# Inuri04/pgtg

Hardware: NVIDIA B200
Metric: env-steps/sec (higher is better)
Workload: dtype int32+f64

## Files before the change

### pgtg_b200/csrc/pgtg_api_impl.hpp

```cpp
#pragma once
#include <math.h>
#include <stdio.h>
#include <stdlib.h>
#include <string.h>

#include <string>
#include <vector>

#include "pgtg_phases.cuh"

using namespace pgtg;

#include "pgtg_env.hpp"

#ifdef PGTG_BACKEND_LEVELS
static const bool bk_has_levels = true;
#else
static const bool bk_has_levels = false;
static int bk_serve_levels(pgtg_env*, void*) { return -1; }
static int bk_levels(pgtg_env*, int32_t*, int, void*) { return -1; }
#endif
#ifdef PGTG_BACKEND_OBS_BITS
static const bool bk_has_obs_bits = true;
#else
// ... 170 lines not shown
  d.visited_penalty = c.already_visited_position_penalty;
  d.ice_p = c.ice_probability; d.broken_p = c.street_damage_probability; d.sand_p = c.sand_probability;
  d.traffic_density = c.traffic_density;
  d.light_green = c.light_green; d.light_yellow = c.light_yellow; d.light_total = c.light_green + c.light_yellow + c.light_red;
  d.ignore_traffic_collisions = c.ignore_traffic_collisions;
  for (int i = 0; i < 5; i++) {
    d.profile_cdf[i] = c.profile_cdf[i]; d.drv_yellow_stop[i] = c.drv_yellow_stop[i]; d.drv_red_violation[i] = c.drv_red_violation[i];
    d.drv_patience_threshold[i] = c.drv_patience_threshold[i]; d.drv_push_probability[i] = c.drv_push_probability[i];
    d.drv_speed_multiplier[i] = c.drv_speed_multiplier[i]; d.drv_reaction_delay[i] = c.drv_reaction_delay[i];
    d.drv_min_following[i] = c.drv_min_following[i];
  }
  d.separate_reward_cost = c.separate_reward_cost; d.num_rules = c.num_rules; d.max_episode_steps = c.max_episode_steps;
  d.write_final_obs = c.write_final_obs;
  for (int i = 0; i < c.num_rules; i++) if (c.rules[i].min_traffic <= 0 && c.rules[i].min_matching_traffic <= 0) d.rules_without_traffic = 1;
  d.max_cars = c.max_cars > 0 ? c.max_cars : 1;
  d.lut_radius = (d.WS > d.HS ? d.WS : d.HS) + 2;
  int words = (d.T + 1) / 2;
  if ((words & 1) == 0) words++;
  d.tile_stride = words * 2;
  for (int t = 0; t < d.T; t++) {
    if (t % d.W < d.W - 1) d.full_e[t >> 5] |= 1u << (t & 31);
    if (t + d.W < d.T) d.full_s[t >> 5] |= 1u << (t & 31);
  }
  if (c.already_visited_position_penalty != 0) { d.vis_w = d.HS + 2; d.vis_words = ((d.WS + 2) * (d.HS + 2) + 31) / 32; }
  d.obs_bits = d.C * d.P * d.P;
  if (c.traffic_density > 0) { d.occ_words = (d.WS * d.HS + 15) / 16;   d.spawner_cap = 2 * (d.W + d.H) + d.T; }
  d.pregen = (c.rng_mode != PGTG_RNG_TAPE && !c.fixed_map) ? 1 : 0;
  d.lean = lean_predicate(c, d);
  d.env_id_base = c.env_id_base; d.seed = c.seed;
  d.num_levels = c.num_levels; d.level_sampling = c.level_sampling; d.start_level = c.start_level;
  if (!c.fixed_map) {
    d.n_edge_tab = 2 * (d.W * (d.H - 1) + d.H * (d.W - 1));
    d.n_border_slots = 2 * d.W + 2 * d.H - 2;
    int n_he = d.H * (d.W - 1), n_ve = d.W * (d.H - 1);
    if (c.start_mode == 0 && c.goal_mode == 0 && d.T <= 32 && n_he + n_ve >= 1 && n_he + n_ve <= bk_conn_table_max_bits() &&
        !(c.start_x == c.goal_x && c.start_y == c.goal_y)) {
      d.conn_bits = n_he + n_ve; d.conn_ne = n_he;
      d.path_tab = d.T <= 16 ? 1 : 0;
    }
    int n_slots = 2 * d.W + 2 * d.H - 2;
    if (c.border_connections < 0 || c.border_connections > n_slots) { why = "random_map_percentage_of_connections must be in [0, 1]"; return -1; }
    if (c.edges_to_keep < 0) { why = "random_map_percentage_of_connections must be in [0, 1]"; return -1; }
  }
  return 0;
}

static int build_level_pool(pgtg_env* e) {
  const size_t M = (size_t)e->cfg.num_levels, T = (size_t)e->dc.T;
  DevPtrs& p = e->dp;
  if (!(p.level_tiles = dev_alloc<uint16_t>(e, M * T + 8, false)) || !(p.level_plan = dev_alloc<uint32_t>(e, M, false))) return -1;
  uint16_t* ring = (uint16_t*)bk_alloc(2 * M * T * 2 + 16);
  uint32_t* plans = (uint32_t*)bk_alloc(2 * M * 4);
  uint64_t* keys = (uint64_t*)bk_alloc(M * 8);
  uint2* list = (uint2*)bk_alloc(2 * M * sizeof(uint2));
  uint32_t* count = (uint32_t*)bk_alloc(8);
  uint32_t* err = (uint32_t*)bk_alloc(M * 4);
  int rc = (ring && plans && keys && list && count && err) ? 0 : -1;
  if (!rc) {
    std::vector<uint64_t> hk(M);
    std::vector<uint2> hl(M);
    for (size_t j = 0; j < M; j++) { hk[j] = (uint64_t)e->cfg.start_level + j; hl[j].x = (uint32_t)j; hl[j].y = 1u; }
    const uint32_t hc[2] = {(uint32_t)M, 0u};
    rc = bk_h2d(keys, hk.data(), M * 8, nullptr) || bk_h2d(list, hl.data(), M * sizeof(uint2), nullptr) || bk_h2d(count, hc, 8, nullptr) ||
         bk_memset(err, 0, M * 4) || bk_sync(nullptr);
  }
  if (!rc) {
// ... 12 lines not shown
    std::vector<uint32_t> hp(M);
    rc = bk_d2d(p.level_tiles, ring + M * T, M * T * 2, nullptr) || bk_d2h(hp.data(), plans + M, M * 4, nullptr) || bk_sync(nullptr);
    for (size_t j = 0; j < M; j++) hp[j] &= ~(3u << 29);
    rc = rc || bk_h2d(p.level_plan, hp.data(), M * 4, nullptr) || bk_sync(nullptr);
  }
  for (void* a : {(void*)ring, (void*)plans, (void*)keys, (void*)list, (void*)count, (void*)err}) if (a) bk_free(a);
  return rc;
}

static int32_t level_fingerprint(const pgtg_config& c) {
  if (!c.num_levels) return 0;
  uint32_t h = 0x9E3779B9u;
  h = (h ^ (uint32_t)c.num_levels) * 0x85EBCA6Bu;
  h = (h ^ (uint32_t)c.start_level) * 0xC2B2AE35u;
  h = (h ^ (uint32_t)c.level_sampling) * 0x27D4EB2Fu;
  return (int32_t)(h | 1u);
}

extern "C" int pgtg_create(const pgtg_config* cfg, int device, pgtg_env** out) {
  if (!cfg || !out) return fail(PGTG_ERR_INVALID, "null argument");
  *out = nullptr;
  DevCfg dc;
  std::string why;
  if (fill_devcfg(*cfg, dc, why)) return fail(PGTG_ERR_INVALID, why);
  if (cfg->num_levels && !bk_has_levels) return fail(PGTG_ERR_INVALID, "num_levels: this backend has no level sets");
  if (bk_set_device(device)) return fail(PGTG_ERR_CUDA, std::string("cannot select device: ") + bk_error());
  pgtg_env* e = new pgtg_env();
  e->cfg = *cfg; e->dc = dc; e->device = device; e->launches = 0;
  e->max_steps_cfg = dc.max_episode_steps; e->gamma_cap = 0;
  e->have_fixed = e->have_tape = e->did_reset = false;
  e->cars_injected = false;
  e->timing = false; e->tev_used = 0;
  e->side_stream = e->ev_tick = e->ev_map[0] = e->ev_map[1] = nullptr;
  e->launch_index = 0; e->mapgen_grid = 0; e->inline_mapgen = false;
  e->flat = nullptr; e->flat_dim = 0;
  e->info_dev = nullptr;
  e->packed_dev = nullptr; e->stage_dev[0] = e->stage_dev[1] = nullptr; e->stage_bytes = 0; e->copy_stream = nullptr;
  e->ev_stage[0] = e->ev_stage[1] = e->ev_copied[0] = e->ev_copied[1] = nullptr; e->host_steps = 0;
  e->obs_format = PGTG_OBS_INT8; e->obs_map_buf = e->f_obs_map_buf = nullptr; e->obs_packed_buf = e->f_obs_packed_buf = nullptr;
  memset(&e->dp, 0, sizeof e->dp);
  if (pick_block(e->dc, &e->block, &e->smem)) { delete e; return fail(PGTG_ERR_INVALID, "observation window too large for shared memory"); }
  e->nblk = (dc.N + e->block - 1) / e->block;
  e->stats_rows = nullptr;
  e->traffic_G = e->traffic_NT = 0;
  const bool wants_traffic_tick = cfg->traffic_density > 0 || ((cfg->sliding || cfg->use_next_subgoal_direction) && !cfg->fixed_map && getenv("PGTG_TRAFFIC_KERNEL_CARFREE"));
  if (cfg->rng_mode == PGTG_RNG_PHILOX && wants_traffic_tick && !getenv("PGTG_NO_TRAFFIC_KERNEL")) bk_traffic_geometry(e->dc, &e->traffic_G, &e->traffic_NT);
  e->stats_nrows = e->nblk;
  if (e->traffic_G > 0 && (dc.N + e->traffic_G - 1) / e->traffic_G > e->stats_nrows) e->stats_nrows = (dc.N + e->traffic_G - 1) / e->traffic_G;
  DevPtrs& p = e->dp;
  size_t N = (size_t)dc.N;
  bool ok = true;
#define A(field, type, count) ok = ok && ((p.field = dev_alloc<type>(e, (count))) != nullptr) && (e->state_allocs.push_back({p.field, sizeof(type) * (size_t)(count)}), true)
  A(agent, short4, N); A(misc, uint32_t, N); A(elapsed, uint32_t, N); A(episode, uint32_t, N); A(next_car_id, uint32_t, N);
  A(plan, uint32_t, N); A(tiles, uint16_t, N * dc.T + 8);
  if (dc.pregen) { A(next_tiles, uint16_t, 2 * N * dc.T + 8); A(next_plan, uint32_t, 2 * N); A(regen_list, uint2, 4 * N); A(regen_count, uint32_t, 4); } A(cars, uint64_t, 2 * (size_t)dc.max_cars * N);
  if (dc.vis_words) A(visited, uint32_t, (size_t)dc.vis_words * N);
  if (dc.occ_words) { A(occ, uint32_t, (size_t)dc.occ_words * N); A(spawners, uint16_t, (size_t)dc.spawner_cap * N); A(spawner_count, uint16_t, N); }
  A(key, uint64_t, N); A(error, uint32_t, N); A(ep_return, double, N);
  if (cfg->rng_mode == PGTG_RNG_TAPE) { A(cursor, int64_t, N); A(tape_end, int64_t, N); }
  if (cfg->rng_mode == PGTG_RNG_NUMPY) { A(pcg, PcgState, 4 * N); p.pcg_stride = N; }
  A(obs_map, int8_t, N * dc.obs_bits + 16); A(obs_position, int32_t, 2 * N); A(obs_velocity, int32_t, 2 * N); A(obs_nsd, int32_t, N);
  A(reward, double, N); A(cost, double, N); A(terminated, uint8_t, N); A(truncated, uint8_t, N);
  A(step_state, int32_t, 4 * N); A(step_flags, uint8_t, N);
  if (dc.write_final_obs) {
    A(f_obs_map, int8_t, N * dc.obs_bits + 16); A(f_obs_position, int32_t, 2 * N); A(f_obs_velocity, int32_t, 2 * N); A(f_obs_nsd, int32_t, N);
  }
  A(stats, double, 8);
// ... 66 lines not shown
          uint8_t& v = tl[((size_t)ex * 81 + sq) * PGTG_NUM_ROUTE_IDS + r];
          if ((l & 7) != 0) v |= (uint8_t)(16u << ((l & 7) - 1));
          for (int i = 0; i < (int)((l >> 3) & 7); i++)
            if ((int)((l >> (6 + 7 * i)) & 31) == r) v |= (uint8_t)(1u << ((l >> (11 + 7 * i)) & 3));
        }
      }
    uint8_t* sd = dev_alloc<uint8_t>(e, sl.size());
    uint8_t* tdv = dev_alloc<uint8_t>(e, tl.size());
    if (!sd || !tdv) { pgtg_destroy(e); return fail(PGTG_ERR_CUDA, "device allocation failed"); }
    bk_h2d(sd, sl.data(), sl.size(), nullptr);
    bk_h2d(tdv, tl.data(), tl.size(), nullptr);
    bk_sync(nullptr);
    p.step_lut = sd; p.target_lut = tdv;
  }
  {
    std::vector<uint8_t> lut;
    build_direction_lut(dc.lut_radius, lut);
    uint8_t* d = dev_alloc<uint8_t>(e, lut.size());
    pgtg_rule* r = dev_alloc<pgtg_rule>(e, PGTG_MAX_RULES);
    if (!d || !r) { pgtg_destroy(e); return fail(PGTG_ERR_CUDA, "device allocation failed"); }
    bk_h2d(d, lut.data(), lut.size(), nullptr);
    bk_h2d(r, cfg->rules, sizeof(pgtg_rule) * PGTG_MAX_RULES, nullptr);
    p.dirlut = d; p.rules = r;
  }
  if (e->dc.pregen) {
    int sms = 0;
    if (bk_side_create(&e->side_stream, &e->ev_tick, &e->ev_map[0], &e->ev_map[1], &sms)) {
      pgtg_destroy(e);
      return fail(PGTG_ERR_CUDA, std::string("cannot create the map-generation stream: ") + bk_error());
    }
    const char* env_ctas = getenv("PGTG_MAPGEN_CTAS_PER_SM");
    int per_sm = env_ctas ? atoi(env_ctas) : 0;
    e->mapgen_grid = per_sm > 0 ? sms * per_sm : 0;
    e->mapgen_grid_overlap = e->mapgen_grid; e->overlap = !getenv("PGTG_NO_OVERLAP");
    e->inline_mapgen = bk_inline_mapgen() && getenv("PGTG_INLINE_MAPGEN") != nullptr && cfg->rng_mode == PGTG_RNG_PHILOX && !getenv("PGTG_NO_LEAN") && !cfg->num_levels;
  }
  if (e->dc.conn_bits) {
    size_t words = ((size_t)1 << e->dc.conn_bits) / 32 + 1;
    uint32_t* t = dev_alloc<uint32_t>(e, words, false);
    if (!t || bk_build_conn_table(e, t)) { pgtg_destroy(e); return fail(PGTG_ERR_CUDA, std::string("connectivity table: ") + bk_error()); }
    p.conn_table = t;
    const int W = e->dc.W, H = e->dc.H, n_he = H * (W - 1);
    std::vector<uint2> ft((size_t)e->dc.conn_bits);
    for (auto& m : ft) m.x = m.y = 0x80000000u;
    auto add = [&](int edge, uint32_t others) { uint2& m = ft[(size_t)edge]; if (m.x == 0x80000000u) m.x = others; else m.y = others; };
    for (int r = 0; r + 1 < H; r++)
      for (int x = 0; x + 1 < W; x++) {
        const int f[4] = {r * (W - 1) + x, (r + 1) * (W - 1) + x, n_he + r * W + x, n_he + r * W + x + 1};
        uint32_t all = 0;
        for (int k = 0; k < 4; k++) all |= 1u << f[k];
        for (int k = 0; k < 4; k++) add(f[k], all & ~(1u << f[k]));
      }
    uint2* fd = dev_alloc<uint2>(e, ft.size());
    if (!fd) { pgtg_destroy(e); return fail(PGTG_ERR_CUDA, "device allocation failed"); }
    bk_h2d(fd, ft.data(), ft.size() * sizeof(uint2), nullptr);
    p.face_tab = fd;
  }
  if (e->dc.path_tab) {
    uint64_t* t = dev_alloc<uint64_t>(e, (size_t)1 << e->dc.conn_bits, false);
    if (!t || bk_build_path_table(e, t)) { pgtg_destroy(e); return fail(PGTG_ERR_CUDA, std::string("path table: ") + bk_error()); }
    p.path_table = t;
  }
  if (!pgtg::map_in_registers(e->dc)) e->inline_mapgen = false;
  if (cfg->num_levels && build_level_pool(e)) { pgtg_destroy(e); return fail(PGTG_ERR_CUDA, std::string("level pool: ") + bk_error()); }
  bk_sync(nullptr);
  *out = e;
// ... 733 lines not shown
```

### pgtg_b200/csrc/pgtg_device.cuh

```cuda
#pragma once
#include <stdint.h>
#include <stdlib.h>

#ifdef __CUDACC__
#include <cuda_runtime.h>
#define PG_HD __device__ __forceinline__
#define PG_HDN static __device__ __noinline__
#define PG_HOSTDEV __host__ __device__ inline
#define PG_MEMBER __device__
#define PG_DEVCONST __device__ const
#define pg_umulhi(a, b) __umulhi((a), (b))
#define pg_ffs(v) __ffs((int)(v))
#define pg_popc(v) __popc((unsigned)(v))
#define pg_clz(v) __clz((int)(v))
#define pg_popcll(v) __popcll((unsigned long long)(v))
#define pg_ldg(p) __ldg(p)
#define pg_dmul(a, b) __dmul_rn((a), (b))
#define pg_dadd(a, b) __dadd_rn((a), (b))
#define pg_ddiv(a, b) __ddiv_rn((a), (b))
#define pg_atomic_or(p, v) atomicOr((p), (v))
#define pg_atomic_add(p, v) atomicAdd((p), (v))
#define pg_atomic_cas(p, o, n) atomicCAS((p), (o), (n))
#define pg_atomic_min(p, v) atomicMin((p), (v))
#define pg_store_streaming(ptr, v) __stcs((ptr), (v))
// ... 101 lines not shown
}
PG_HOSTDEV unsigned car_xy(uint64_t v) { return (unsigned)(v & 0xFFFF); }

struct DevCfg {
  int N, W, H, T, WS, HS;
  int C, P, sliding, window_k, use_nsd;
  int channel_kind[PGTG_MAX_CHANNELS];
  int kind_channel[16];
  int lean;
  int obs_fast;
  int fixed_map, edges_to_keep, n_edge_tab, border_connections, n_border_slots;
  int start_mode, goal_mode, start_x, start_y, start_dir, goal_x, goal_y, goal_dir, min_sg_dist;
  double obstacle_probability, obstacle_cdf[4];
  double sum_subgoals_reward, final_goal_bonus, crash_penalty, light_penalty, standing_penalty, visited_penalty;
  double ice_p, broken_p, sand_p, traffic_density;
  int light_green, light_yellow, light_total, ignore_traffic_collisions;
  double profile_cdf[5], drv_yellow_stop[5], drv_red_violation[5], drv_patience_threshold[5], drv_push_probability[5],
      drv_speed_multiplier[5], drv_reaction_delay[5];
  int drv_min_following[5];
  int separate_reward_cost, num_rules, max_episode_steps, write_final_obs, max_cars, lut_radius;
  int pregen;
  int rules_without_traffic;
  int tile_stride;
  int vis_w, vis_words;
  int occ_words, spawner_cap;
  int obs_bits;
  uint32_t full_e[8], full_s[8];
  int conn_bits, conn_ne;
  int path_tab;
  int eval_on, gamma_len;
  int64_t env_id_base;
  uint64_t seed;
  int num_levels, level_sampling, start_level;
};

struct PcgState {
  uint64_t st_lo, st_hi, inc_lo, inc_hi;
  uint32_t buf, has;
};

struct Lut;

struct DevPtrs {
  short4* agent;
  uint32_t* misc;
  uint32_t* elapsed;
  uint32_t* episode;
  uint32_t* next_car_id;
  uint32_t* plan;
  uint16_t* tiles;
  uint16_t* next_tiles;
  uint32_t* next_plan;
  uint2* regen_list;
  uint32_t* regen_count;
  int parity;
  uint64_t* cars;
  uint32_t* visited;
  uint32_t* occ;
  uint16_t* spawners;
  uint16_t* spawner_count;
  uint64_t* key;
  PcgState* pcg;
  size_t pcg_stride;
  int64_t* cursor;
  int64_t* tape_end;
  const double* tape_values;
// ... 406 lines not shown
```

### pgtg_b200/csrc/pgtg_env.hpp

```cpp
#pragma once
#include <stdint.h>

#include <vector>

#include "pgtg_phases.cuh"

using namespace pgtg;

namespace pgtg { constexpr int STATS_STRIDE = 8; }

enum { MODE_STEP = 0, MODE_RESET = 1, MODE_OBSERVE = 2, MODE_MAPGEN = 3 };

struct pgtg_env {
  pgtg_config cfg;
  DevCfg dc;
  DevPtrs dp;
  int device;
  int block;
  size_t smem;
  int64_t launches;
  std::vector<void*> allocs;
  struct StateAlloc { void* ptr; size_t bytes; };
  std::vector<StateAlloc> state_allocs;
  bool have_fixed, have_tape, did_reset;
  int max_steps_cfg;
  int gamma_cap;
  bool cars_injected;
  int nblk;
  int stats_nrows;
  int traffic_G, traffic_NT;
  void* side_stream; void* ev_tick; void* ev_map[2];
  uint64_t launch_index;
  bool inline_mapgen;
  int mapgen_grid;
  int mapgen_grid_overlap; bool overlap;
  bool timing; std::vector<void*> tev; int tev_used;
  float* flat; int flat_dim; int flat_order[PGTG_MAX_CHANNELS];
  uint32_t* packed_dev; unsigned char* stage_dev[2]; size_t stage_bytes; void* copy_stream; void* ev_stage[2]; void* ev_copied[2]; uint64_t host_steps;
  int obs_format; int8_t* obs_map_buf; int8_t* f_obs_map_buf; uint32_t* obs_packed_buf; uint32_t* f_obs_packed_buf;
  uint32_t* unpack_err;
  int32_t* info_dev;
  double* stats_rows;
  uint8_t* mask_dev;
  int64_t* seeds_dev;
  int32_t* actions_dev;
  std::vector<uint16_t> edge_tab, edge_rev, border_slots;
};

static inline bool inline_mapgen_now(const pgtg_env* e) { return e->inline_mapgen && e->dc.pregen && e->dc.lean == 1 && !e->dc.write_final_obs; }
```

### pgtg_b200/csrc/pgtg_logic.cuh

```cuda
#pragma once
#include "pgtg_device.cuh"

namespace pgtg {

PG_HD int select32(uint32_t v, int n);

PG_HD uint64_t* car_list(const DevCfg& c, const DevPtrs& p, int env, int half) { return p.cars + ((size_t)env * 2 + half) * c.max_cars; }

PG_HD int light_phase(const DevCfg& c, int counter) {
  return counter < c.light_green ? 0 : (counter < c.light_green + c.light_yellow ? 1 : 2);
}

PG_HD void or_bit81(uint32_t w[3], int sq) {
  uint32_t b = 1u << (sq & 31);
  int i = sq >> 5;
  w[0] |= i == 0 ? b : 0u; w[1] |= i == 1 ? b : 0u; w[2] |= i == 2 ? b : 0u;
}

PG_HD void spawner_bits(const DevCfg& c, const Lut& L, int ex, int tx, int ty, uint32_t out[3]) {
  out[0] = out[1] = out[2] = 0;
  if (ex == 0) return;
  int ns = L.native_spawner[ex];
  if (ns != 255) or_bit81(out, ns);
  if (tx == 0) { int sq = L.entry_sq[3]; if (ld_all(lane_desc(ex, sq)) == 4) or_bit81(out, sq); }
// ... 585 lines not shown

template <int RNG>
PG_HD uint32_t remove_edges_tabled(const DevCfg& c, const DevPtrs& p, Rng<RNG>& rng, uint8_t* arr) {
  const int n_und = c.H * (c.W - 1) + c.W * (c.H - 1);
  uint32_t graph = (c.conn_bits >= 32 ? 0u : (1u << c.conn_bits)) - 1u;
  for (int i = 0; 4 * i < n_und; i++) ((uint32_t*)arr)[i] = 0x03020100u + 0x04040404u * (uint32_t)i;
  int n = n_und;
  int go = n > 0 ? 2 * n_und - c.edges_to_keep : 0;
  uint32_t pos = rng.position(PGTG_STREAM_MAP);
  while (go > 0) {
    uint32_t w[4];
    rng.block(PGTG_STREAM_MAP, pos >> 2, w);
#pragma unroll
    for (int k = 0; k < 4; k++) {
      if (go > 0) {
        const int i = (int)pg_umulhi(w[k], (uint32_t)n);
        const int edge = arr[i];
        const uint32_t pbit = 1u << edge;
        arr[i] = arr[n - 1];
        n--; pos++;
        const uint32_t g2 = graph & ~pbit;
        const uint2 face = pg_ldg(&p.face_tab[edge]);
        bool keep = (graph & face.x) == face.x || (graph & face.y) == face.y;
        if (!keep) keep = (pg_ldg(&p.conn_table[g2 >> 5]) >> (g2 & 31)) & 1u;
        graph = keep ? g2 : graph;
        go = n > 0 ? 2 * pg_popc(graph) - c.edges_to_keep : 0;
      }
    }
  }
  rng.set_position(PGTG_STREAM_MAP, pos);
  return graph;
}

template <int RNG, typename MASK = uint64_t>
PG_HD MASK choose_border_slots(const DevCfg& c, Rng<RNG>& rng) {
  const int n = c.n_border_slots;
  int left = c.border_connections < n ? c.border_connections : n;
  MASK chosen = 0;
  if (left <= 0) return chosen;
  const int cbits = edge_chunk_bits(n), per_word = 32 / cbits;
  const uint32_t cmask = (1u << cbits) - 1u;
  const MASK valid = n >= (int)(8 * sizeof(MASK)) ? ~(MASK)0 : (((MASK)1 << n) - 1);
  while (left > 0) {
    uint32_t cw = rng.word(PGTG_STREAM_MAP);
    for (int k = 0; k < per_word && left > 0; k++) {
      const MASK bit = (MASK)1 << (cw & cmask);
      cw >>= cbits;
      if (bit & valid & ~chosen) { chosen |= bit; left--; }
    }
  }
  return chosen;
}

template <int RNG>
PG_HD unsigned obstacle_draw(const DevCfg& c, Rng<RNG>& rng, int ex) {
  const double u = rng.uniform(PGTG_STREAM_MAP);
  if (!(u < c.obstacle_probability) || ex == 0) return 0u;
  const int type = 1 + rng.choice_cdf(PGTG_STREAM_MAP, c.obstacle_cdf, 4);
  int mask;
  if (type != 4) mask = rng.index(PGTG_STREAM_MAP, 8);
  else {
    const int cnt = pg_popc(ex);
    unsigned cand = (unsigned)(ex & 15);
    if ((ex & 1) && (ex & 4) && cnt >= 3) cand |= 16u;
    if ((ex & 2) && (ex & 8) && cnt >= 3) cand |= 32u;
    int k = rng.index(PGTG_STREAM_MAP, pg_popc(cand));
    while (k-- > 0) cand &= cand - 1;
    mask = 8 + pg_ffs(cand) - 1;
  }
  return (unsigned)(type << 4 | mask << 7);
}

template <int RNG, int TMAX, bool TABLED = false>
PG_HD void generate_map(const DevCfg& c, const DevPtrs& p, MapView& m, EnvRegs& e, Rng<RNG>& rng) {
  int sx = c.start_x, sy = c.start_y, sd = c.start_dir, gx = c.goal_x, gy = c.goal_y, gd = c.goal_dir;
  if (!TABLED && (c.start_mode != 0 || c.goal_mode != 0)) choose_start_goal<RNG>(c, rng, sx, sy, sd, gx, gy, gd);
  int W = c.W, T = c.T;
  int st = sy * W + sx, gt = gy * W + gx;

  Board<TMAX> E, S;
#pragma unroll
// ... 215 lines not shown
  return v;
}

PG_HOSTDEV int plan_start_index(unsigned pl) { return (pl >> 29) & 3; }

template <int RNG, int TMAX, bool TABLED = false, bool POOL = true>
PG_HD void build_map(const DevCfg& c, const DevPtrs& p, MapView& m, EnvRegs& e, Rng<RNG>& rng) {
  if (POOL && RNG == PGTG_RNG_PHILOX && c.num_levels) {
    uint32_t w1;
    const uint32_t lv = level_draw(c, p.key[rng.env], e.episode, rng.env, &w1);
    for (int t = 0; t < c.T; t++) m.tiles[t] = pg_ldg(&p.level_tiles[(size_t)lv * c.T + t]);
    e.plan = pg_ldg(&p.level_plan[lv]);
    if (start_line_labelled(m.tiles[plan_sy(e.plan) * c.W + plan_sx(e.plan)], e.plan)) e.plan |= pg_umulhi(w1, 3u) << 29;
    else e.err |= 64;
    m.plan = e.plan;
    return;
  }
  if (!TABLED && c.fixed_map) {
    for (int t = 0; t < c.T; t++) m.tiles[t] = pg_ldg(&p.fixed_tiles[t]);
    e.plan = p.fixed_plan;
  } else {
    generate_map<RNG, TMAX, TABLED>(c, p, m, e, rng);
  }
  assign_subgoals<TMAX, TABLED>(c, p, m, e);
  m.plan = e.plan;
  int stile = m.start_tile(), sd = plan_sd(e.plan);
  unsigned lab = (m.line_labels(stile, m.tiles[stile]) >> (4 * sd)) & 15;
  if (lab == 3) e.plan |= (unsigned)rng.index(PGTG_STREAM_MAP, 3) << 29;
  else e.err |= 64;
  m.plan = e.plan;
}

PG_HOSTDEV bool map_in_registers(const DevCfg& c) {
  return c.conn_bits != 0 && c.path_tab && (c.T == 8 || c.T == 16) && c.start_mode == 0 && c.goal_mode == 0 && !c.fixed_map;
}
template <int RNG>
PG_HD void build_map_in_registers(const DevCfg& c, const DevPtrs& p, EnvRegs& e, Rng<RNG>& rng, uint8_t* arr, uint32_t* dst ) {
  const uint32_t graph = remove_edges_tabled<RNG>(c, p, rng, arr);
  const uint64_t v = pg_ldg(&p.path_table[graph]);
  uint32_t E, S;
  graph_to_boards(c, graph, E, S);
  const uint32_t Sn = S << c.W, Ew = E << 1;
  const int st = c.start_y * c.W + c.start_x, gt = c.goal_y * c.W + c.goal_x;
  uint64_t border = (uint64_t)(1u << c.start_dir) << (4 * st) | (uint64_t)(1u << c.goal_dir) << (4 * gt);
  for (uint32_t chosen = choose_border_slots<RNG, uint32_t>(c, rng); chosen != 0u; chosen &= chosen - 1u) {
    const unsigned s = pg_ldg(&p.border_slots[pg_ffs(chosen) - 1]);
    border |= (uint64_t)(1u << (s >> 8)) << (4 * (s & 255u));
  }
  if (c.obstacle_probability > 0) {
    for (int k = 0; 2 * k < c.T; k++) {
      uint32_t w = 0;
      for (int h = 0; h < 2; h++) {
        const int t = 2 * k + h;
        const uint32_t ex = ((Sn >> t) & 1u) | ((E >> t) & 1u) << 1 | ((S >> t) & 1u) << 2 | ((Ew >> t) & 1u) << 3 | ((uint32_t)(border >> (4 * t)) & 15u);
        const uint32_t sg = (uint32_t)(v >> (3 * t)) & 7u;
        w |= (ex | obstacle_draw<RNG>(c, rng, (int)ex) | sg << 11) << (16 * h);
      }
      dst[k] = w;
    }
  } else {
    const uint32_t sg_lo = (uint32_t)v, sg_hi = (uint32_t)(v >> 24);
    const uint32_t bd_lo = (uint32_t)border, bd_hi = (uint32_t)(border >> 32);
    uint32_t out[8];
#pragma unroll
    for (int k = 0; k < 8; k++) {
      uint32_t w = 0;
#pragma unroll
      for (int h = 0; h < 2; h++) {
        const int t = 2 * k + h;
        const uint32_t ex = ((Sn >> t) & 1u) | ((E >> t) & 1u) << 1 | ((S >> t) & 1u) << 2 | ((Ew >> t) & 1u) << 3 | (((t < 8 ? bd_lo : bd_hi) >> (4 * (t & 7))) & 15u);
        const uint32_t sg = ((t < 8 ? sg_lo : sg_hi) >> (3 * (t & 7))) & 7u;
        w |= (ex | sg << 11) << (16 * h);
      }
      out[k] = w;
    }
    { uint4 q; q.x = out[0]; q.y = out[1]; q.z = out[2]; q.w = out[3]; ((uint4*)dst)[0] = q; }
    if (c.T == 16) { uint4 q; q.x = out[4]; q.y = out[5]; q.z = out[6]; q.w = out[7]; ((uint4*)dst)[1] = q; }
  }
// ... 268 lines not shown
```

### pgtg_b200/csrc/pgtg_phases.cuh

```cuda
#pragma once
#include "pgtg_logic.cuh"

namespace pgtg {

struct BlockShared {
  Lut* lut;
  EnvRegs* regs;
  uint16_t* tiles;
  int* done_list;
  int* counters;
  double* dsum;
  uint32_t* bits;
  int bits_words;
  uint2* spread;
  uint16_t* edge_tab;
  uint16_t* edge_rev;
  uint16_t* border_slots;
};

PG_HOSTDEV size_t align16(size_t v) { return (v + 15) & ~(size_t)15; }
PG_HOSTDEV int block_bits_words(const DevCfg& c, int B) { return (B * c.obs_bits + 31) / 32 + 4; }
PG_HOSTDEV size_t block_shared_bytes(const DevCfg& c, int B, bool lean = false) {
  return align16(sizeof(Lut)) + (lean ? 0 : align16(sizeof(EnvRegs) * B)) + align16(sizeof(uint16_t) * B * c.tile_stride) +
         (lean ? 0 : align16(sizeof(int) * B)) + align16(sizeof(int) * 40) + align16(sizeof(double) * 8) +
// ... 156 lines not shown
  if (PREGEN) env_reset_pregenerated<RNG, LEAN>(c, p, m, e, env);
  else env_reset<RNG, TMAX>(c, p, m, e, env);
}
template <int RNG, int TMAX, bool PREGEN, bool LEAN = false>
PG_HD void phase_reset(const DevCfg& c, const DevPtrs& p, const BlockShared& sh, int local, int env) {
  EnvRegs e = sh.regs[local];
  phase_reset_regs<RNG, TMAX, PREGEN, LEAN>(c, p, sh, local, env, e);
  sh.regs[local] = e;
}

template <int RNG, int TMAX, bool TABLED = false>
PG_HD void phase_pregenerate(const DevCfg& c, const DevPtrs& p, const BlockShared& sh, int tid, int env, uint32_t episode) {
  EnvRegs e;
  e.x = e.y = e.vx = e.vy = 0; e.misc = 0; e.next_car_id = 0; e.plan = 0; e.err = 0; e.cursor = 0; e.flags = 0;
  e.elapsed = 0;
  e.episode = episode;
  MapView m = {c, *sh.lut, sh.tiles + tid * c.tile_stride, 0u, sh.edge_tab, sh.edge_rev, sh.border_slots, 0u, false};
  Rng<RNG> rng(p, e, env);
  build_map<RNG, TMAX, TABLED, false>(c, p, m, e, rng);
  rng.flush();
  const size_t slot = episode & 1u;
  uint16_t* nt = p.next_tiles + (slot * c.N + (size_t)env) * c.T;
  if ((c.T & 7) == 0) {
    const uint32_t* s32 = (const uint32_t*)m.tiles;
    uint4* g4 = (uint4*)nt;
    for (int k = 0; k < c.T / 8; k++) { uint4 v; v.x = s32[4 * k]; v.y = s32[4 * k + 1]; v.z = s32[4 * k + 2]; v.w = s32[4 * k + 3]; g4[k] = v; }
  } else {
    for (int t = 0; t < c.T; t++) nt[t] = m.tiles[t];
  }
  p.next_plan[slot * c.N + env] = e.plan;
  if (e.err) p.error[env] |= e.err;
}

template <int RNG>
PG_HD void phase_pregenerate_in_registers(const DevCfg& c, const DevPtrs& p, uint8_t* arr, int env, uint32_t episode) {
  EnvRegs e;
  e.x = e.y = e.vx = e.vy = 0; e.misc = 0; e.next_car_id = 0; e.plan = 0; e.err = 0; e.cursor = 0; e.flags = 0;
  e.elapsed = 0;
  e.episode = episode;
  Rng<RNG> rng(p, e, env);
  const size_t slot = episode & 1u;
  build_map_in_registers<RNG>(c, p, e, rng, arr, (uint32_t*)(p.next_tiles + (slot * c.N + (size_t)env) * c.T));
  p.next_plan[slot * c.N + env] = e.plan;
  if (e.err) p.error[env] |= e.err;
}

PG_HD void phase_serve_level(const DevCfg& c, const DevPtrs& p, int env, uint32_t episode) {
  uint32_t w1;
  const uint32_t lv = level_draw(c, pg_ldg(&p.key[env]), episode, env, &w1);
  const size_t slot = episode & 1u;
  const uint16_t* src = p.level_tiles + (size_t)lv * c.T;
  uint16_t* dst = p.next_tiles + (slot * c.N + (size_t)env) * c.T;
  if ((c.T & 7) == 0) {
    for (int k = 0; k < c.T / 8; k++) ((uint4*)dst)[k] = pg_ldg((const uint4*)src + k);
  } else {
    for (int t = 0; t < c.T; t++) dst[t] = pg_ldg(&src[t]);
  }
  unsigned plan = pg_ldg(&p.level_plan[lv]);
  if (start_line_labelled(pg_ldg(&src[plan_sy(plan) * c.W + plan_sx(plan)]), plan)) plan |= pg_umulhi(w1, 3u) << 29;
  else p.error[env] |= 64;
  p.next_plan[slot * c.N + env] = plan;
}

PG_HD int32_t env_level(const DevCfg& c, const DevPtrs& p, int env, int previous) {
  uint32_t w1;
  return (int32_t)level_draw(c, p.key[env], p.episode[env] - (uint32_t)previous, env, &w1);
}

template <bool LEAN, bool SLIDE = false>
PG_HD void write_obs_scalars_and_state(const DevCfg& c, const DevPtrs& p, const uint16_t* tiles_sh, int env, const EnvRegs& e,
                                       const int32_t* pos, const int32_t* vel, int32_t nsd);
template <bool LEAN = false, bool SLIDE = false>
PG_HD void phase_emit_regs(const DevCfg& c, const DevPtrs& p, const BlockShared& sh, int tid, int env, bool final_obs, const EnvRegs& e) {
  MapView m = {c, *sh.lut, sh.tiles + tid * c.tile_stride, e.plan, sh.edge_tab, sh.edge_rev, sh.border_slots, 0u, false};
  int32_t pos[2], vel[2], nsd;
// ... 212 lines not shown
```

### pgtg_b200/csrc/pgtg_tick_kernels.cuh

```cuda
#pragma once
#include <cuda_runtime.h>
#include <stdio.h>
#include <stdlib.h>

#include "pgtg_env.hpp"

namespace pgtg {

#ifndef PGTG_MIN_BLOCKS
#define PGTG_MIN_BLOCKS 8
#endif
#ifndef PGTG_MAPGEN_TABLED_MIN_BLOCKS
#define PGTG_MAPGEN_TABLED_MIN_BLOCKS 12
#endif
#ifndef PGTG_LEAN_MIN_BLOCKS
#define PGTG_LEAN_MIN_BLOCKS 8
#endif
#define PGTG_EDGE_ROW 28
#ifndef PGTG_MAPGEN_MIN_BLOCKS
#define PGTG_MAPGEN_MIN_BLOCKS 12
#endif

struct StatsArgs {
  double* rows;
// ... 76 lines not shown
          uint4 z; z.x = z.y = z.z = z.w = 0;
          uint4* b4 = (uint4*)sh.bits;
          for (int i = tid; i < sh.bits_words / 4; i += B) b4[i] = z;
          for (int i = (sh.bits_words / 4) * 4 + tid; i < sh.bits_words; i += B) sh.bits[i] = 0;
        }
        __syncthreads();
      }
      if (done) {
        if (LEAN) { k = er.episode + 1u; phase_reset_regs<RNG, TMAX, true, true>(c, p, sh, tid, env, er); }
        else { k = sh.regs[tid].episode + 1u; phase_reset<RNG, TMAX, true, false>(c, p, sh, tid, env); }
      }
      PG_CLK(4)
      if (valid) { if (LEAN) phase_emit_regs<true, SLIDE>(c, p, sh, tid, env, false, er); else phase_emit<false>(c, p, sh, tid, env, false); }
      PG_CLK(5)
      if (!INLINE && any) {
        qbase = __shfl_sync(0xffffffffu, qbase, 0);
        if (done) {
          uint2 q; q.x = (uint32_t)env; q.y = k + 2u;
          p.regen_list[(size_t)p.parity * 2 * c.N + qbase + __popc(any & ((1u << lane) - 1u))] = q;
        }
      }
      PG_CLK(6)
      __syncthreads();
      PG_CLK(7)
      if (tid == 0 && sh.counters[12]) {
        double* row = sa.rows + (size_t)blockIdx.x * STATS_STRIDE;
        row[0] += sh.counters[12]; row[1] += sh.dsum[0]; row[2] += sh.counters[11];
        row[3] += sh.counters[8]; row[4] += sh.counters[9]; row[5] += sh.counters[10];
        if (c.eval_on) { row[6] += sh.dsum[1]; row[7] += sh.counters[13]; }
      }
      phase_expand(c, p.obs_map, sh, tid, B, env0, nvalid, p.obs_packed);
      PG_CLK(8)
      if (INLINE && LEAN && done)
        phase_pregenerate_in_registers<RNG>(c, p, (uint8_t*)(sh.tiles + tid * c.tile_stride), env, k + 2u);
      return;
    }
  } else if (MODE == MODE_RESET) {
    if (valid) {
      EnvRegs e = load_regs(c, p, env);
      if (!mask || mask[env]) {
        if (seeds) { p.key[env] = (uint64_t)seeds[env]; e.episode = 0; }
        p.ep_return[env] = 0.0;
        if (p.ep_disc) p.ep_disc[env] = 0.0;
        done = true;
      }
      sh.regs[tid] = e;
    }
  } else {
    if (valid) sh.regs[tid] = load_regs(c, p, env);
  }

  if (LEAN) return;

  unsigned ballot = __ballot_sync(0xffffffffu, done);
  if (lane == 0) sh.counters[1 + warp] = __popc(ballot);
  __syncthreads();
  int base = 0, n_done = 0;
  for (int w = 0; w < nwarps; w++) { int v = sh.counters[1 + w]; if (w < warp) base += v; n_done += v; }
  if (done) sh.done_list[base + __popc(ballot & ((1u << lane) - 1u))] = tid;
  if (MODE == MODE_STEP && tid == 0 && n_done) {
    double* row = sa.rows + (size_t)blockIdx.x * STATS_STRIDE;
    row[0] += n_done; row[1] += sh.dsum[0]; row[2] += sh.counters[11];
    row[3] += sh.counters[8]; row[4] += sh.counters[9]; row[5] += sh.counters[10];
    if (c.eval_on) { row[6] += sh.dsum[1]; row[7] += sh.counters[13]; }
  }
  __syncthreads();

// ... 22 lines not shown

  if (MODE != MODE_OBSERVE) {
    if (tid < n_done) {
      int local = sh.done_list[tid];
      phase_reset<RNG, TMAX, PREGEN>(c, p, sh, local, env0 + local);
    }
    __syncthreads();
  }
  if (valid) phase_emit(c, p, sh, tid, env, false);
  __syncthreads();
  phase_expand(c, p.obs_map, sh, tid, B, env0, nvalid, p.obs_packed);
}

template <int RNG, int TMAX, bool TABLED = false>
__global__ void __launch_bounds__(128, TABLED ? PGTG_MAPGEN_TABLED_MIN_BLOCKS : PGTG_MAPGEN_MIN_BLOCKS) pgtg_mapgen_kernel(const __grid_constant__ DevCfg c, const __grid_constant__ DevPtrs p, int parity,
                                                                                const __grid_constant__ SharedLayout layout) {
  extern __shared__ __align__(16) unsigned char smem[];
  const uint32_t count = p.regen_count[parity];
  if (blockIdx.x * blockDim.x >= count) return;
  const uint2* list = p.regen_list + (size_t)parity * 2 * c.N;
  BlockShared sh = carve_layout(smem, layout);
  stage_tables(c, p, sh, threadIdx.x, blockDim.x);
  __syncthreads();
  for (uint32_t i = blockIdx.x * blockDim.x + threadIdx.x; i < count; i += gridDim.x * blockDim.x) {
    uint2 r = list[i];
    phase_pregenerate<RNG, TMAX, TABLED>(c, p, sh, threadIdx.x, (int)r.x, r.y);
  }
}

template <int RNG, int MINB>
__global__ void __launch_bounds__(128, MINB) pgtg_mapgen_registers_kernel(const __grid_constant__ DevCfg c, const __grid_constant__ DevPtrs p, int parity) {
  extern __shared__ __align__(16) unsigned char smem[];
  const uint32_t count = p.regen_count[parity];
  if (blockIdx.x * blockDim.x >= count) return;
  const uint2* list = p.regen_list + (size_t)parity * 2 * c.N;
  for (uint32_t i = blockIdx.x * blockDim.x + threadIdx.x; i < count; i += gridDim.x * blockDim.x) {
    const uint2 r = list[i];
    phase_pregenerate_in_registers<RNG>(c, p, smem + threadIdx.x * PGTG_EDGE_ROW, (int)r.x, r.y);
  }
}

}

static inline int lk(cudaError_t e) { return (int)e; }

template <int RNG, int MODE, int TMAX, bool PREGEN, bool LEAN = false, bool FINAL = false, bool SLIDE = false, bool INLINE = false>
static int launch_one(pgtg_env* e, const uint8_t* mask, const int64_t* seeds, const void* actions, int action_bytes, cudaStream_t st) {
  auto kern = pgtg::pgtg_tick_kernel<RNG, MODE, TMAX, PREGEN, LEAN, FINAL, SLIDE, INLINE>;
  static bool carve_set = false;
  const size_t smem = LEAN ? pgtg::block_shared_bytes(e->dc, e->block, true) : e->smem;
  if (!carve_set) {
    const bool fits164 = LEAN && (smem + 1024) * PGTG_LEAN_MIN_BLOCKS <= 164u * 1024u;
    const char* cv = getenv("PGTG_TICK_CARVEOUT");
    cudaFuncSetAttribute(kern, cudaFuncAttributePreferredSharedMemoryCarveout, cv ? atoi(cv) : fits164 ? 72 : (int)cudaSharedmemCarveoutMaxShared);
    carve_set = true;
  }
  if (smem > 48 * 1024) {
    { int rc = lk(cudaFuncSetAttribute(kern, cudaFuncAttributeMaxDynamicSharedMemorySize, (int)smem)); if (rc) return rc; }
  }
  pgtg::StatsArgs sa = {e->stats_rows};
  unsigned char* const origin = (unsigned char*)4096;
  const pgtg::SharedLayout layout = pgtg::layout_of(pgtg::carve_shared(origin, e->dc, e->block, LEAN), origin);
  kern<<<e->nblk, e->block, smem, st>>>(e->dc, e->dp, mask, seeds, actions, action_bytes, sa, layout);
  return lk(cudaGetLastError());
}

template <int RNG, int MODE, bool PREGEN>
static int launch_sized(pgtg_env* e, const uint8_t* mask, const int64_t* seeds, const void* actions, int action_bytes, cudaStream_t st) {
  if (e->dc.T <= 16) return launch_one<RNG, MODE, 16, PREGEN>(e, mask, seeds, actions, action_bytes, st);
  if (e->dc.T <= 64) return launch_one<RNG, MODE, 64, PREGEN>(e, mask, seeds, actions, action_bytes, st);
  return launch_one<RNG, MODE, 256, PREGEN>(e, mask, seeds, actions, action_bytes, st);
}

template <int RNG, int MINB>
static int launch_mapgen_registers(pgtg_env* e, cudaStream_t st, int grid, int carveout) {
  auto kern = pgtg::pgtg_mapgen_registers_kernel<RNG, MINB>;
  static bool carve_set = false;
  if (!carve_set) { cudaFuncSetAttribute(kern, cudaFuncAttributePreferredSharedMemoryCarveout, carveout); carve_set = true; }
  kern<<<grid, 128, 128 * PGTG_EDGE_ROW, st>>>(e->dc, e->dp, e->dp.parity);
  return lk(cudaGetLastError());
}

template <int RNG, int TMAX, bool TABLED = false>
static int launch_mapgen(pgtg_env* e, cudaStream_t st) {
  const int B = 128;
  size_t smem = pgtg::mapgen_shared_bytes(e->dc, B);
  int full = (2 * e->dc.N + B - 1) / B;
  int grid = e->mapgen_grid > 0 && e->mapgen_grid < full ? e->mapgen_grid : full;
  if constexpr (RNG == PGTG_RNG_PHILOX && TABLED) {
    if (pgtg::map_in_registers(e->dc) && !getenv("PGTG_NO_MAP_IN_REGISTERS")) {
      const char* mb = getenv("PGTG_MAPGEN_MINB");
      const char* cv = getenv("PGTG_MAPGEN_CARVEOUT");
      const int minb = mb ? atoi(mb) : 12, carve = cv ? atoi(cv) : (e->traffic_G > 0 ? (int)cudaSharedmemCarveoutMaxShared : 30);
      if (minb >= 16) return launch_mapgen_registers<RNG, 16>(e, st, grid, carve);
      if (minb >= 12) return launch_mapgen_registers<RNG, 12>(e, st, grid, carve);
      if (minb >= 10) return launch_mapgen_registers<RNG, 10>(e, st, grid, carve);
      return launch_mapgen_registers<RNG, 8>(e, st, grid, carve);
    }
  }
  auto kern = pgtg::pgtg_mapgen_kernel<RNG, TMAX, TABLED>;
  static bool carve_set = false;
  if (!carve_set) { cudaFuncSetAttribute(kern, cudaFuncAttributePreferredSharedMemoryCarveout, cudaSharedmemCarveoutMaxShared); carve_set = true; }
  if (smem > 48 * 1024) { int rc = lk(cudaFuncSetAttribute(kern, cudaFuncAttributeMaxDynamicSharedMemorySize, (int)smem)); if (rc) return rc; }
  unsigned char* const origin = (unsigned char*)4096;
  const pgtg::SharedLayout layout = pgtg::layout_of(pgtg::carve_mapgen(origin, e->dc, B), origin);
  kern<<<grid, B, smem, st>>>(e->dc, e->dp, e->dp.parity, layout);
  return lk(cudaGetLastError());
}

template <int RNG>
static int launch_mode(pgtg_env* e, int mode, const uint8_t* mask, const int64_t* seeds, const void* actions, int action_bytes, cudaStream_t st) {
  switch (mode) {
    case MODE_STEP:
      if (RNG != PGTG_RNG_TAPE && e->dc.pregen && e->dc.lean && !getenv("PGTG_NO_LEAN")) {
        constexpr int R = RNG == PGTG_RNG_TAPE ? PGTG_RNG_PHILOX : RNG;
        constexpr bool L = RNG != PGTG_RNG_TAPE;
        if (e->dc.lean == 2) {
          if (e->dc.write_final_obs) return launch_one<R, MODE_STEP, 16, L, L, L, L>(e, mask, seeds, actions, action_bytes, st);
          return launch_one<R, MODE_STEP, 16, L, L, false, L>(e, mask, seeds, actions, action_bytes, st);
        }
        if (e->dc.write_final_obs) return launch_one<R, MODE_STEP, 16, L, L, L>(e, mask, seeds, actions, action_bytes, st);
        if constexpr (RNG == PGTG_RNG_PHILOX) { if (inline_mapgen_now(e)) return launch_one<R, MODE_STEP, 16, L, L, false, false, L>(e, mask, seeds, actions, action_bytes, st); }
        return launch_one<R, MODE_STEP, 16, L, L>(e, mask, seeds, actions, action_bytes, st);
      }
      if (RNG != PGTG_RNG_TAPE && e->dc.pregen) return launch_sized<RNG, MODE_STEP, RNG != PGTG_RNG_TAPE>(e, mask, seeds, actions, action_bytes, st);
      return launch_sized<RNG, MODE_STEP, false>(e, mask, seeds, actions, action_bytes, st);
    case MODE_RESET:
      return launch_sized<RNG, MODE_RESET, false>(e, mask, seeds, actions, action_bytes, st);
    case MODE_MAPGEN:
      if (RNG == PGTG_RNG_TAPE) return (int)cudaErrorInvalidValue;
// ... 10 lines not shown
```

Measured before the change: 4.618 billion.

## Pair edge removals per RNG block and size register mapgen grid by occupancy

```diff
diff --git a/pgtg_b200/csrc/pgtg_api_impl.hpp b/pgtg_b200/csrc/pgtg_api_impl.hpp
--- a/pgtg_b200/csrc/pgtg_api_impl.hpp
+++ b/pgtg_b200/csrc/pgtg_api_impl.hpp
@@ -226,6 +226,7 @@
   if (!c.fixed_map) {
     d.n_edge_tab = 2 * (d.W * (d.H - 1) + d.H * (d.W - 1));
     d.n_border_slots = 2 * d.W + 2 * d.H - 2;
+    d.border_bits = (int16_t)pgtg::edge_chunk_bits(d.n_border_slots); d.border_per_word = (int16_t)(32 / d.border_bits);
     int n_he = d.H * (d.W - 1), n_ve = d.W * (d.H - 1);
     if (c.start_mode == 0 && c.goal_mode == 0 && d.T <= 32 && n_he + n_ve >= 1 && n_he + n_ve <= bk_conn_table_max_bits() &&
         !(c.start_x == c.goal_x && c.start_y == c.goal_y)) {
@@ -304,7 +305,7 @@
   e->cars_injected = false;
   e->timing = false; e->tev_used = 0;
   e->side_stream = e->ev_tick = e->ev_map[0] = e->ev_map[1] = nullptr;
-  e->launch_index = 0; e->mapgen_grid = 0; e->inline_mapgen = false;
+  e->launch_index = 0; e->mapgen_grid = 0; e->sm_count = 0; e->inline_mapgen = false;
   e->flat = nullptr; e->flat_dim = 0;
   e->info_dev = nullptr;
   e->packed_dev = nullptr; e->stage_dev[0] = e->stage_dev[1] = nullptr; e->stage_bytes = 0; e->copy_stream = nullptr;
@@ -437,6 +438,7 @@
     const char* env_ctas = getenv("PGTG_MAPGEN_CTAS_PER_SM");
     int per_sm = env_ctas ? atoi(env_ctas) : 0;
     e->mapgen_grid = per_sm > 0 ? sms * per_sm : 0;
+    e->sm_count = sms;
     e->mapgen_grid_overlap = e->mapgen_grid; e->overlap = !getenv("PGTG_NO_OVERLAP");
     e->inline_mapgen = bk_inline_mapgen() && getenv("PGTG_INLINE_MAPGEN") != nullptr && cfg->rng_mode == PGTG_RNG_PHILOX && !getenv("PGTG_NO_LEAN") && !cfg->num_levels;
   }
diff --git a/pgtg_b200/csrc/pgtg_device.cuh b/pgtg_b200/csrc/pgtg_device.cuh
--- a/pgtg_b200/csrc/pgtg_device.cuh
+++ b/pgtg_b200/csrc/pgtg_device.cuh
@@ -157,6 +157,7 @@
   int64_t env_id_base;
   uint64_t seed;
   int num_levels, level_sampling, start_level;
+  int16_t border_bits, border_per_word;
 };
 
 struct PcgState {
diff --git a/pgtg_b200/csrc/pgtg_env.hpp b/pgtg_b200/csrc/pgtg_env.hpp
--- a/pgtg_b200/csrc/pgtg_env.hpp
+++ b/pgtg_b200/csrc/pgtg_env.hpp
@@ -33,6 +33,7 @@
   uint64_t launch_index;
   bool inline_mapgen;
   int mapgen_grid;
+  int sm_count;
   int mapgen_grid_overlap; bool overlap;
   bool timing; std::vector<void*> tev; int tev_used;
   float* flat; int flat_dim; int flat_order[PGTG_MAX_CHANNELS];
diff --git a/pgtg_b200/csrc/pgtg_logic.cuh b/pgtg_b200/csrc/pgtg_logic.cuh
--- a/pgtg_b200/csrc/pgtg_logic.cuh
+++ b/pgtg_b200/csrc/pgtg_logic.cuh
@@ -641,6 +641,51 @@
   return graph;
 }
 
+PG_HD bool face_intact(uint32_t graph, uint2 face) { return (graph & face.x) == face.x || (graph & face.y) == face.y; }
+template <int RNG>
+PG_HD uint32_t remove_edges_paired(const DevCfg& c, const DevPtrs& p, Rng<RNG>& rng, uint8_t* arr) {
+  const int n_und = c.H * (c.W - 1) + c.W * (c.H - 1);
+  uint32_t graph = (c.conn_bits >= 32 ? 0u : (1u << c.conn_bits)) - 1u;
+  for (int i = 0; 4 * i < n_und; i++) ((uint32_t*)arr)[i] = 0x03020100u + 0x04040404u * (uint32_t)i;
+  int n = n_und, score = 2 * n_und - c.edges_to_keep;
+  const uint32_t pos0 = rng.position(PGTG_STREAM_MAP);
+  while (n > 0 && score > 0) {
+    uint32_t w[4];
+    rng.block(PGTG_STREAM_MAP, (pos0 + (uint32_t)(n_und - n)) >> 2, w);
+#pragma unroll
+    for (int k = 0; k < 4; k += 2) {
+      if (n > 0 && score > 0) {
+        const int ia = (int)pg_umulhi(w[k], (uint32_t)n);
+        const int ea = arr[ia];
+        arr[ia] = arr[n - 1];
+        const int nb = n > 1 ? n - 1 : 1;
+        const int ib = (int)pg_umulhi(w[k + 1], (uint32_t)nb);
+        const int eb = arr[ib];
+        arr[ib] = arr[nb - 1];
+        const uint2 fa = pg_ldg(&p.face_tab[ea]), fb = pg_ldg(&p.face_tab[eb]);
+        const uint32_t ga = graph & ~(1u << ea);
+        const uint32_t gk = ga & ~(1u << eb), gr = graph & ~(1u << eb);
+        uint32_t wa = ~0u, wk = ~0u, wr = ~0u;
+        if (!face_intact(graph, fa)) wa = pg_ldg(&p.conn_table[ga >> 5]);
+        if (!face_intact(ga, fb)) wk = pg_ldg(&p.conn_table[gk >> 5]);
+        if (!face_intact(graph, fb)) wr = pg_ldg(&p.conn_table[gr >> 5]);
+        const bool keep_a = (wa >> (ga & 31)) & 1u;
+        graph = keep_a ? ga : graph;
+        score -= keep_a ? 2 : 0;
+        n--;
+        if (n > 0 && score > 0) {
+          const bool keep_b = keep_a ? (wk >> (gk & 31)) & 1u : (wr >> (gr & 31)) & 1u;
+          graph = keep_b ? (keep_a ? gk : gr) : graph;
+          score -= keep_b ? 2 : 0;
+          n--;
+        }
+      }
+    }
+  }
+  rng.set_position(PGTG_STREAM_MAP, pos0 + (uint32_t)(n_und - n));
+  return graph;
+}
+
 template <int RNG, typename MASK = uint64_t>
 PG_HD MASK choose_border_slots(const DevCfg& c, Rng<RNG>& rng) {
   const int n = c.n_border_slots;
@@ -656,6 +701,25 @@
       const MASK bit = (MASK)1 << (cw & cmask);
       cw >>= cbits;
       if (bit & valid & ~chosen) { chosen |= bit; left--; }
+    }
+  }
+  return chosen;
+}
+template <int RNG>
+PG_HD uint32_t choose_border_slots_regs(const DevCfg& c, Rng<RNG>& rng) {
+  const int n = c.n_border_slots, cbits = c.border_bits, per_word = c.border_per_word;
+  int left = c.border_connections < n ? c.border_connections : n;
+  const uint32_t cmask = (1u << cbits) - 1u, valid = n >= 32 ? ~0u : (1u << n) - 1u;
+  uint32_t chosen = 0;
+  while (left > 0) {
+    uint32_t cw = rng.word(PGTG_STREAM_MAP);
+#pragma unroll
+    for (int k = 0; k < 8; k++) {
+      const uint32_t bit = (1u << (cw & cmask)) & valid & ~chosen;
+      const bool take = bit != 0u && left > 0 && k < per_word;
+      chosen |= take ? bit : 0u;
+      left -= take ? 1 : 0;
+      cw >>= cbits;
     }
   }
   return chosen;
@@ -937,18 +1001,19 @@
 }
 
 PG_HOSTDEV bool map_in_registers(const DevCfg& c) {
-  return c.conn_bits != 0 && c.path_tab && (c.T == 8 || c.T == 16) && c.start_mode == 0 && c.goal_mode == 0 && !c.fixed_map;
-}
-template <int RNG>
+  return c.conn_bits != 0 && c.path_tab && (c.T == 8 || c.T == 16) && c.start_mode == 0 && c.goal_mode == 0 && !c.fixed_map &&
+         c.border_per_word <= 8;
+}
+template <int RNG, bool PAIRED = true>
 PG_HD void build_map_in_registers(const DevCfg& c, const DevPtrs& p, EnvRegs& e, Rng<RNG>& rng, uint8_t* arr, uint32_t* dst ) {
-  const uint32_t graph = remove_edges_tabled<RNG>(c, p, rng, arr);
+  const uint32_t graph = PAIRED ? remove_edges_paired<RNG>(c, p, rng, arr) : remove_edges_tabled<RNG>(c, p, rng, arr);
   const uint64_t v = pg_ldg(&p.path_table[graph]);
   uint32_t E, S;
   graph_to_boards(c, graph, E, S);
   const uint32_t Sn = S << c.W, Ew = E << 1;
   const int st = c.start_y * c.W + c.start_x, gt = c.goal_y * c.W + c.goal_x;
   uint64_t border = (uint64_t)(1u << c.start_dir) << (4 * st) | (uint64_t)(1u << c.goal_dir) << (4 * gt);
-  for (uint32_t chosen = choose_border_slots<RNG, uint32_t>(c, rng); chosen != 0u; chosen &= chosen - 1u) {
+  for (uint32_t chosen = PAIRED ? choose_border_slots_regs<RNG>(c, rng) : choose_border_slots<RNG, uint32_t>(c, rng); chosen != 0u; chosen &= chosen - 1u) {
     const unsigned s = pg_ldg(&p.border_slots[pg_ffs(chosen) - 1]);
     border |= (uint64_t)(1u << (s >> 8)) << (4 * (s & 255u));
   }
diff --git a/pgtg_b200/csrc/pgtg_phases.cuh b/pgtg_b200/csrc/pgtg_phases.cuh
--- a/pgtg_b200/csrc/pgtg_phases.cuh
+++ b/pgtg_b200/csrc/pgtg_phases.cuh
@@ -212,7 +212,7 @@
   if (e.err) p.error[env] |= e.err;
 }
 
-template <int RNG>
+template <int RNG, bool PAIRED = true>
 PG_HD void phase_pregenerate_in_registers(const DevCfg& c, const DevPtrs& p, uint8_t* arr, int env, uint32_t episode) {
   EnvRegs e;
   e.x = e.y = e.vx = e.vy = 0; e.misc = 0; e.next_car_id = 0; e.plan = 0; e.err = 0; e.cursor = 0; e.flags = 0;
@@ -220,7 +220,7 @@
   e.episode = episode;
   Rng<RNG> rng(p, e, env);
   const size_t slot = episode & 1u;
-  build_map_in_registers<RNG>(c, p, e, rng, arr, (uint32_t*)(p.next_tiles + (slot * c.N + (size_t)env) * c.T));
+  build_map_in_registers<RNG, PAIRED>(c, p, e, rng, arr, (uint32_t*)(p.next_tiles + (slot * c.N + (size_t)env) * c.T));
   p.next_plan[slot * c.N + env] = e.plan;
   if (e.err) p.error[env] |= e.err;
 }
diff --git a/pgtg_b200/csrc/pgtg_tick_kernels.cuh b/pgtg_b200/csrc/pgtg_tick_kernels.cuh
--- a/pgtg_b200/csrc/pgtg_tick_kernels.cuh
+++ b/pgtg_b200/csrc/pgtg_tick_kernels.cuh
@@ -132,7 +132,7 @@
       phase_expand(c, p.obs_map, sh, tid, B, env0, nvalid, p.obs_packed);
       PG_CLK(8)
       if (INLINE && LEAN && done)
-        phase_pregenerate_in_registers<RNG>(c, p, (uint8_t*)(sh.tiles + tid * c.tile_stride), env, k + 2u);
+        phase_pregenerate_in_registers<RNG, false>(c, p, (uint8_t*)(sh.tiles + tid * c.tile_stride), env, k + 2u);
       return;
     }
   } else if (MODE == MODE_RESET) {
@@ -221,7 +221,6 @@
 __global__ void __launch_bounds__(128, MINB) pgtg_mapgen_registers_kernel(const __grid_constant__ DevCfg c, const __grid_constant__ DevPtrs p, int parity) {
   extern __shared__ __align__(16) unsigned char smem[];
   const uint32_t count = p.regen_count[parity];
-  if (blockIdx.x * blockDim.x >= count) return;
   const uint2* list = p.regen_list + (size_t)parity * 2 * c.N;
   for (uint32_t i = blockIdx.x * blockDim.x + threadIdx.x; i < count; i += gridDim.x * blockDim.x) {
     const uint2 r = list[i];
@@ -262,11 +261,18 @@
 }
 
 template <int RNG, int MINB>
-static int launch_mapgen_registers(pgtg_env* e, cudaStream_t st, int grid, int carveout) {
+static int launch_mapgen_registers(pgtg_env* e, cudaStream_t st, int grid, int full, int carveout) {
   auto kern = pgtg::pgtg_mapgen_registers_kernel<RNG, MINB>;
-  static bool carve_set = false;
-  if (!carve_set) { cudaFuncSetAttribute(kern, cudaFuncAttributePreferredSharedMemoryCarveout, carveout); carve_set = true; }
-  kern<<<grid, 128, 128 * PGTG_EDGE_ROW, st>>>(e->dc, e->dp, e->dp.parity);
+  const size_t smem = 128 * PGTG_EDGE_ROW;
+  static int per_sm = 0;
+  if (!per_sm) {
+    cudaFuncSetAttribute(kern, cudaFuncAttributePreferredSharedMemoryCarveout, carveout);
+    { int rc = lk(cudaOccupancyMaxActiveBlocksPerMultiprocessor(&per_sm, kern, 128, smem)); if (rc) return rc; }
+    if (per_sm < 1) per_sm = 1;
+  }
+  if (grid <= 0) grid = e->sm_count * per_sm;
+  if (grid > full) grid = full;
+  kern<<<grid, 128, smem, st>>>(e->dc, e->dp, e->dp.parity);
   return lk(cudaGetLastError());
 }
 
@@ -281,10 +287,11 @@
       const char* mb = getenv("PGTG_MAPGEN_MINB");
       const char* cv = getenv("PGTG_MAPGEN_CARVEOUT");
       const int minb = mb ? atoi(mb) : 12, carve = cv ? atoi(cv) : (e->traffic_G > 0 ? (int)cudaSharedmemCarveoutMaxShared : 30);
-      if (minb >= 16) return launch_mapgen_registers<RNG, 16>(e, st, grid, carve);
-      if (minb >= 12) return launch_mapgen_registers<RNG, 12>(e, st, grid, carve);
-      if (minb >= 10) return launch_mapgen_registers<RNG, 10>(e, st, grid, carve);
-      return launch_mapgen_registers<RNG, 8>(e, st, grid, carve);
+      const int pgrid = e->mapgen_grid;
+      if (minb >= 16) return launch_mapgen_registers<RNG, 16>(e, st, pgrid, full, carve);
+      if (minb >= 12) return launch_mapgen_registers<RNG, 12>(e, st, pgrid, full, carve);
+      if (minb >= 10) return launch_mapgen_registers<RNG, 10>(e, st, pgrid, full, carve);
+      return launch_mapgen_registers<RNG, 8>(e, st, pgrid, full, carve);
     }
   }
   auto kern = pgtg::pgtg_mapgen_kernel<RNG, TMAX, TABLED>;
```

Result: slower. 4.528 billion, median of 6 (-1.9%).
